# xuhaocuhk/TilinGNN

Measured on AMD Instinct MI355X. Metric: scored tile-nodes/sec (GNN forward), higher is better.
Workload: dtype f32; 1 GPU; TilinGNN.forward on a seeded banded super-graph: 100000 nodes / 1000000 adjacency edges / 1250000 collision edges per GPU, tile_count 2, T=13 edge types, width 32, depth 20, train-mode BatchNorm, graph prep included; n_nodes=100000, n_adj_edges=1000000, n_col_edges=1250000, parallelism=single GPU

## Files before the change

tilingnn_amd/_lib.py:

```python
from __future__ import annotations

import ctypes as C
import os

_HERE = os.path.dirname(os.path.abspath(__file__))
LIB_PATH = os.environ.get("TGNN_LIB_PATH") or os.path.join(_HERE, "libtgnn.so")

ACT_NONE, ACT_LEAKY_RELU, ACT_SIGMOID = 0, 1, 2
BN_MAX_PARTIALS = 512
BN_STAT_ROWS = 4


class TgnnError(RuntimeError):
    code = 0


class ModelDims(C.Structure):
    _fields_ = [("node_features_dim", C.c_int32), ("adj_edge_features_dim", C.c_int32),
                ("network_width", C.c_int32), ("network_depth", C.c_int32), ("output_dim", C.c_int32)]


class Graph(C.Structure):
    _fields_ = [("n_nodes", C.c_int64), ("n_adj_edges", C.c_int64), ("n_col_edges", C.c_int64),
                ("n_types", C.c_int32),
# ... 184 lines not shown
                                           p]),
        "tgnn_nnconv_type_sum": (C.c_int, [p, i64, p, i64, p, p, p, p, i64, i32, i32, p, p]),
        "tgnn_csr_degree": (C.c_int, [p, i64, p, p, p]),
        "tgnn_unsupervised_loss_bwd": (C.c_int, [p, i64, p, i64, i64, p, i64, p, i64, p, i64, f32, f32, f32, p, p, p, i64,
                                                 p, sz, p]),
        "tgnn_f32_to_bf16": (C.c_int, [p, i64, p, p]),
        "tgnn_nnconv64_image_elems": (sz, [i32]),
        "tgnn_nnconv64_bf16_fwd": (C.c_int, [p, i64, p, p, p, p, i32, p, p, i64, i32, p, p, p, pi32, p]),
        "tgnn_nnconv64_bf16_eg_fwd": (C.c_int, [p, i64, p, p, p, i32, p, p, i64, i32, p, p, p, pi32, p]),
        "tgnn_gin64_bf16_fwd": (C.c_int, [p, p, p, p, p, p, p, p, p, p, p, i64, i32, p, p, p, pi32, p]),
        "tgnn_collconv64_bf16_fwd": (C.c_int, [p, p, p, p, p, p, p, p, p, p, p, p, p, p, p, i64, p, p, p, p, p, p]),
        "tgnn_merge_bf16_fwd": (C.c_int, [p, p, p, p, p, i64, i32, p, p]),
        "tgnn_dense_bf16_slots_fwd": (C.c_int, [p, i64, i32, p, p, i64, i32, i32, p, p, p, pi32, p]),
        "tgnn_forward_bf16_workspace_bytes": (sz, [C.POINTER(ModelDims), i64, i32]),
        "tgnn_forward_bf16": (C.c_int, [C.POINTER(ModelDims), C.POINTER(C.c_void_p), p, p, C.POINTER(Graph), i32, p, p, sz, p, p]),
        "tgnn_forward_bf16_begin": (C.c_int, [C.POINTER(ModelDims), C.POINTER(C.c_void_p), p, i64, i32, p, sz, p]),
        "tgnn_rows_gather": (C.c_int, [p, i64, p, i64, i32, p, i64, p]),
        "tgnn_rows_scatter": (C.c_int, [p, p, i64, i32, p, i64, p]),
    }
    for name, (res, args) in sigs.items():
        fn = getattr(lib, name)
        fn.restype, fn.argtypes = res, args
    for name, (res, args) in {"tgnn_debug_spin_fault": (None, [i32]), "tgnn_debug_set_csr_bucket_cap": (i32, [i32]),
                              "tgnn_debug_set_block_caps": (None, [i32, i32])}.items():
        try:
            fn = getattr(lib, name)
        except AttributeError:
            continue
        fn.restype, fn.argtypes = res, args
    return lib


DEBUG_LIB_PATH = os.path.join(_HERE, "libtgnn_debug.so")


def has_debug_hooks() -> bool:
    return hasattr(lib, "tgnn_debug_spin_fault")


lib = _load()
EXPORTED_SYMBOLS = (
    "tgnn_version", "tgnn_last_error", "tgnn_csr_workspace_bytes", "tgnn_csr_build",
    "tgnn_edge_dedup_workspace_bytes", "tgnn_edge_type_dedup", "tgnn_gather_i32", "tgnn_edge_weight_table",
    "tgnn_nnconv_mean_fwd", "tgnn_nnconv_cols_max_columns", "tgnn_nnconv_cols_workspace_bytes",
    "tgnn_nnconv_cols_build", "tgnn_nnconv_cols_max_types", "tgnn_nnconv_weight_image_floats", "tgnn_nnconv_mean_cols_fwd", "tgnn_nnconv_mean_cols_f16_fwd", "tgnn_nnconv_eg_max_groups", "tgnn_nnconv_eg_build", "tgnn_nnconv_mean_eg_fwd",
    "tgnn_ubench_row_gather", "tgnn_mid_entries_words", "tgnn_mid_entries_build", "tgnn_forward_path_counts", "tgnn_set_mid_layout_limit", "tgnn_get_mid_layout_limit", "tgnn_mid_layout_max_nodes",
    "tgnn_spin_error_poll", "tgnn_set_spin_budget_us", "tgnn_persist_fallback", "tgnn_spin_error_peek", "tgnn_gin_fwd", "tgnn_dense_act_fwd", "tgnn_dense_act_slots_fwd", "tgnn_dense_act_slots_f16_fwd", "tgnn_bn_finalize", "tgnn_bn_apply",
# ... 207 lines not shown
```

tilingnn_amd/csrc/graph_prep.hip:

```cpp
#include <atomic>
#include <chrono>
#include <mutex>
#include <vector>

#include "tgnn_common.h"

namespace tgnn {

constexpr int kScanThreads = 256;
constexpr int kScanItems = 8;
constexpr int kScanTile = kScanThreads * kScanItems;

__device__ __forceinline__ int wave_inclusive_scan(int v) {
    const int lane = threadIdx.x & 63;
#pragma unroll
    for (int d = 1; d < 64; d <<= 1) {
        int t = __shfl_up(v, d, 64);
        if (lane >= d) v += t;
    }
    return v;
}

__global__ __launch_bounds__(kScanThreads) void scan_tiles_kernel(const int *in, int *out,
                                                                  int *__restrict__ block_sums, int64_t n) {
// ... 478 lines not shown
    const int n_edge_cols = base[k][n_types];
    for (int c = 0; c < n_edge_cols; ++c) col_slot_src[(c0 + c) * 16 + i] = -1;
    for (int t = i; t < n_types; t += 16) {
        const int m = maxm[k][t];
        for (int r = 0; r < m; ++r)
            col_meta[c0 + base[k][t] + r] = t | (r == 0 ? 1 << 8 : 0) | (r == m - 1 ? 1 << 9 : 0);
    }
    const int deg = e1 - e0;
    col_slot_src[(c0 + n_edge_cols) * 16 + i] = row < n ? __float_as_int((float)(deg > 0 ? deg : 1)) : -1;
    if (i == 0) col_meta[c0 + n_edge_cols] = n_types | (1 << 8) | (1 << 9) | (1 << 10);
    __builtin_amdgcn_fence(__ATOMIC_RELEASE, "wavefront");
    __builtin_amdgcn_wave_barrier();
    for (int t = 0; t < n_types; ++t) cnt[tid][t] = 0;
    for (int e = e0; e < e1; ++e) {
        const int t = col_type[e];
        const int r = cnt[tid][t]++;
        col_slot_src[(c0 + base[k][t] + r) * 16 + i] = col_src[e];
    }
}

constexpr int kEgRoot = 1 << 8;
constexpr int kPrepWordsMagic = 0x600D0001;

template <bool FILL>
__global__ __launch_bounds__(64) void nnconv_eg_kernel(const int *__restrict__ rowptr, const int *__restrict__ col_src,
                                                       const int *__restrict__ col_type, int64_t n, int n_types_host,
                                                       int *__restrict__ tile_grps,
                                                       const int *__restrict__ tile_grp_ptr,
                                                       int2 *__restrict__ grp,
                                                       const int *__restrict__ n_types_dev = nullptr, int max_types = kMaxColTypes,
                                                       int *__restrict__ built_flag = nullptr,
                                                       const int *__restrict__ edge_type = nullptr,
                                                       const int *__restrict__ col_eid = nullptr,
                                                       int *__restrict__ col_type_out = nullptr,
                                                       const int *__restrict__ result_words = nullptr,
                                                       int *__restrict__ host_words = nullptr) {
    if (!FILL && host_words && blockIdx.x == 0 && threadIdx.x < 32) {
        const int v = result_words[threadIdx.x];
        if (threadIdx.x < 31) __hip_atomic_store(host_words + threadIdx.x, v, __ATOMIC_RELAXED, __HIP_MEMORY_SCOPE_SYSTEM);
        __threadfence_system();
        if (threadIdx.x == 31) __hip_atomic_store(host_words + 31, kPrepWordsMagic, __ATOMIC_RELEASE, __HIP_MEMORY_SCOPE_SYSTEM);
    }
    const int n_types = n_types_dev ? *n_types_dev : n_types_host;
    const int64_t n_tiles = (n + kColTileRows - 1) / kColTileRows;
    if (!FILL && col_type_out) {
        const int64_t row0 = (int64_t)blockIdx.x * 64 + threadIdx.x;
        if (row0 < n)
            for (int e = rowptr[row0]; e < rowptr[row0 + 1]; ++e) col_type_out[e] = edge_type[col_eid[e]];
    }
    if (!FILL && blockIdx.x == 0 && threadIdx.x == 0) tile_grps[n_tiles] = 0;
    const int tid = threadIdx.x, k = tid >> 4, i = tid & 15;
    const int64_t row = (int64_t)blockIdx.x * 64 + tid;
    const int64_t tile = (int64_t)blockIdx.x * 4 + k;
    if (n_types > max_types || n_types > kMaxColTypes) {
        if (!FILL && i == 0 && tile < n_tiles) tile_grps[tile] = 0;
        return;
    }
    if (built_flag && blockIdx.x == 0 && threadIdx.x == 0) *built_flag = 1;
    __shared__ unsigned short cnt[64][kMaxColTypes + 1];
    __shared__ unsigned short pre[FILL ? 64 : 1][kMaxColTypes + 1];
    __shared__ int base[4][kMaxColTypes + 1];
    for (int t = 0; t < n_types; ++t) cnt[tid][t] = 0;
    int e0 = 0, e1 = 0;
    if (row < n) { e0 = rowptr[row]; e1 = rowptr[row + 1]; }
    if (!FILL && col_type_out) {
        for (int e = e0; e < e1; ++e) cnt[tid][col_type_out[e]]++;
    } else {
        for (int e = e0; e < e1; ++e) cnt[tid][col_type[e]]++;
    }
    __syncthreads();
    for (int t = i; t < n_types; t += 16) {
        int acc = 0;
        for (int r = 0; r < 16; ++r) {
            if constexpr (FILL) pre[k * 16 + r][t] = (unsigned short)acc;
            acc += cnt[k * 16 + r][t];
        }
        base[k][t] = (acc + 15) >> 4;
    }
    __syncthreads();
    if (i == 0) {
        int acc = 0;
        for (int t = 0; t < n_types; ++t) { const int g = base[k][t]; base[k][t] = acc; acc += g; }
        base[k][n_types] = acc;
        if (!FILL && tile < n_tiles) tile_grps[tile] = acc + 1;
    }
    if (!FILL) return;
    __syncthreads();
    if (tile >= n_tiles) return;
    const int64_t g0 = tile_grp_ptr[tile];
    const int n_edge_grps = base[k][n_types];
    for (int t = 0; t < n_types; ++t)
        for (int g = base[k][t]; g < base[k][t + 1]; ++g) grp[(g0 + g) * 16 + i] = make_int2(-1, t << 16);
    const int deg = e1 - e0;
    grp[(g0 + n_edge_grps) * 16 + i] =
        make_int2(row < n ? __float_as_int((float)(deg > 0 ? deg : 1)) : -1, (n_types | kEgRoot) << 16 | 1 << i);
    __builtin_amdgcn_fence(__ATOMIC_RELEASE, "wavefront");
    __builtin_amdgcn_wave_barrier();
    for (int t = 0; t < n_types; ++t) {
        const int c = cnt[tid][t];
        if (c == 0) continue;
        const int p0 = pre[tid][t], p1 = p0 + c;
        for (int g = p0 >> 4; g <= (p1 - 1) >> 4; ++g) {
            const int lo = max(p0 - 16 * g, 0), hi = min(p1 - 16 * g, 16);
            grp[(g0 + base[k][t] + g) * 16 + i].y = t << 16 | (((1 << hi) - 1) & ~((1 << lo) - 1));
        }
        cnt[tid][t] = 0;
    }
    for (int e = e0; e < e1; ++e) {
        const int t = col_type[e];
        const int p = (unsigned short)(pre[tid][t] + cnt[tid][t]++);
        grp[(g0 + base[k][t] + (p >> 4)) * 16 + (p & 15)].x = col_src[e];
    }
}

constexpr int kSmallPrepThreads = 1024, kSmallPrepMaxNodes = 4096, kSmallPrepMaxBlocks = 16;
constexpr int kSmallPrepLocal = 8192;
constexpr int kSmallPrepGlobal = 8192;
constexpr int kSmallPrepMaxTypes = 1024;

struct SmallPrepArgs {
    const int64_t *adj_ei, *col_ei;
    const float *attr;
    int64_t n, ea, ec;
    int fe, max_col_types;
    int *adj_rowptr, *adj_src, *adj_eid, *adj_type;
    int *edge_type, *type_rep;
    int *col_rowptr, *col_src, *col_eid;
    int *tile_col_ptr, *col_meta, *col_slot_src;
    int *result_host;
    int *tmp;
    int *result;
    unsigned *ctr;
};

__device__ int small_block_scan(int *a, int m, int *wave_tot) {
// ... 421 lines not shown

constexpr int kBkLogMax = 9, kBkRows = 1 << kBkLogMax, kBkMaxBuckets = 4096, kBkThreads = 1024;
constexpr int kBkCap = 15360;
constexpr int kBkCapHalf = 7168;
struct BkSet {
    const int64_t *ei;
    int64_t e;
    int drop_self;
    int *rowptr, *col_src, *col_eid, *err_flag;
    int *rec_eid, *rec_src;
    unsigned short *rec_row;
    int *total_out, *max_deg_out;
};
struct BkArgs {
    BkSet set[2];
    int64_t n, n_src;
    int nb, nblk;
    int lg;
    int cap;
    int cap_lds;
    int *hist;
    const int *tile_off;
    unsigned *scan_ticket;
};
__device__ __forceinline__ int bk_scanned(const BkArgs &A, int64_t i) {
    const int v = A.hist[i];
    return A.tile_off ? v + A.tile_off[i / kScanTile] : v;
}

__global__ __launch_bounds__(kBkThreads) void bk_hist_kernel(BkArgs A) {
    extern __shared__ int bk_h[];
    const BkSet S = A.set[blockIdx.y];
    const int tid = threadIdx.x, blk = blockIdx.x;
    for (int b = tid; b < A.nb; b += kBkThreads) bk_h[b] = 0;
    __syncthreads();
    const int64_t i0 = S.e * blk / A.nblk, i1 = S.e * (blk + 1) / A.nblk;
    for (int64_t i = i0 + tid; i < i1; i += kBkThreads) {
        const int64_t s = S.ei[i], d = S.ei[S.e + i];
        if (s < 0 || s >= A.n_src || d < 0 || d >= A.n) {
            if (S.err_flag) *S.err_flag = 1;
        } else if (!(S.drop_self && s == d)) {
            atomicAdd(&bk_h[d >> A.lg], 1);
        }
    }
    __syncthreads();
    for (int b = tid; b < A.nb; b += kBkThreads) A.hist[((int64_t)blockIdx.y * A.nb + b) * A.nblk + blk] = bk_h[b];
    if (blk == 0 && blockIdx.y == 1 && tid == 0) {
        A.hist[(int64_t)2 * A.nb * A.nblk] = 0;
        if (A.scan_ticket) *A.scan_ticket = 0u;
    }
}

constexpr int kBkChunk = kBkThreads * 8;
__global__ __launch_bounds__(kBkThreads) void bk_scatter_kernel(BkArgs A) {
    extern __shared__ int bk_h[];
    int *cur = bk_h, *lcnt = cur + A.nb, *lstart = lcnt + A.nb, *wtot = lstart + A.nb;
    int *l_eid = wtot + 16, *l_src = l_eid + kBkChunk;
    unsigned short *l_row = reinterpret_cast<unsigned short *>(l_src + kBkChunk), *l_bkt = l_row + kBkChunk;
    const BkSet S = A.set[blockIdx.y];
    const int tid = threadIdx.x, blk = blockIdx.x;
    const int base = bk_scanned(A, (int64_t)blockIdx.y * A.nb * A.nblk);
    for (int b = tid; b < A.nb; b += kBkThreads) cur[b] = bk_scanned(A, ((int64_t)blockIdx.y * A.nb + b) * A.nblk + blk) - base;
    const int64_t i0 = S.e * blk / A.nblk, i1 = S.e * (blk + 1) / A.nblk;
    const int per = (A.nb + kBkThreads - 1) / kBkThreads;
    for (int64_t c0 = i0; c0 < i1; c0 += kBkChunk) {
        for (int b = tid; b < A.nb; b += kBkThreads) lcnt[b] = 0;
        __syncthreads();
        int e_b[8], e_r[8], e_s[8], e_row[8];
#pragma unroll
        for (int u = 0; u < 8; ++u) {
            const int64_t i = c0 + tid + (int64_t)u * kBkThreads;
            e_b[u] = -1;
// ... 208 lines not shown
    hipEvent_t ev = nullptr;
    TGNN_CHECK_HIP(prep_words_event(&ev));
    TGNN_CHECK_HIP(hipEventSynchronize(ev));
    return TGNN_OK;
}

static int bk_blocks(int64_t e_max) {
    int64_t nblk = (e_max + 8191) / 8192;
    return (int)(nblk < 1 ? 1 : (nblk > 256 ? 256 : nblk));
}
static int bk_log_rows(int64_t n, int64_t e_max) {
    return (n <= (int64_t)256 * kBkMaxBuckets && e_max * 256 <= (int64_t)3584 * (n > 0 ? n : 1)) ? 8 : 9;
}
static size_t bk_workspace_bytes(int64_t n, int64_t ea, int64_t ec) {
    const int64_t rows = (int64_t)1 << bk_log_rows(n, ea > ec ? ea : ec);
    const int64_t nb = (n + rows - 1) / rows, nblk = bk_blocks(ea > ec ? ea : ec), cells = 2 * nb * nblk + 1;
    return align_up((size_t)cells * 4, 256) + scan_ws_ints(cells) * 4 + align_up((size_t)(ea > 0 ? ea : 1) * 10, 256) +
           align_up((size_t)(ec > 0 ? ec : 1) * 10, 256) + 2048;
}
static bool bk_fits(int64_t n) { return (n + kBkRows - 1) / kBkRows <= kBkMaxBuckets; }

static int csr_build_pair_bucketed(const int64_t *adj_ei, int64_t ea, const int64_t *col_ei, int64_t ec, int64_t n, int64_t n_src,
                                   int *a_rowptr, int *a_src, int *a_eid, int *a_err, int *c_rowptr, int *c_src, int *c_eid,
                                   int *c_err, int *a_max_deg, int *c_total, void *ws, size_t ws_bytes, hipStream_t s) {
    BkArgs A{};
    A.n = n; A.n_src = n_src;
    A.lg = bk_log_rows(n, ea > ec ? ea : ec);
    A.nb = (int)((n + ((int64_t)1 << A.lg) - 1) >> A.lg);
    A.nblk = bk_blocks(ea > ec ? ea : ec);
    A.cap_lds = A.lg == 8 ? kBkCapHalf : kBkCap;
    A.cap = g_bk_cap.load() < A.cap_lds ? g_bk_cap.load() : A.cap_lds;
    const int64_t cells = (int64_t)2 * A.nb * A.nblk + 1;
    Carver cv(ws, ws_bytes);
    A.hist = cv.take<int>(cells);
    int *scan_ws = cv.take<int>(scan_ws_ints(cells));
    const int64_t es[2] = {ea, ec};
    for (int k = 0; k < 2; ++k) {
        const int64_t e1 = es[k] > 0 ? es[k] : 1;
        unsigned char *rec = cv.take<unsigned char>((size_t)e1 * 10);
        A.set[k].rec_eid = reinterpret_cast<int *>(rec);
        A.set[k].rec_src = reinterpret_cast<int *>(rec + (size_t)e1 * 4);
        A.set[k].rec_row = reinterpret_cast<unsigned short *>(rec + (size_t)e1 * 8);
    }
    A.set[0].ei = adj_ei; A.set[0].e = ea; A.set[0].drop_self = 0;
    A.set[0].rowptr = a_rowptr; A.set[0].col_src = a_src; A.set[0].col_eid = a_eid; A.set[0].err_flag = a_err;
    A.set[1].ei = col_ei; A.set[1].e = ec; A.set[1].drop_self = 1;
    A.set[1].rowptr = c_rowptr; A.set[1].col_src = c_src; A.set[1].col_eid = c_eid; A.set[1].err_flag = c_err;
    A.set[0].max_deg_out = a_max_deg;
// ... 8 lines not shown
    bk_hist_kernel<<<dim3(A.nblk, 2), kBkThreads, lds_h, s>>>(A);
    if (fused_scan)
        scan_tiles_fused_kernel<<<(unsigned)scan_tiles, kScanThreads, 0, s>>>(A.hist, A.hist, scan_ws, const_cast<int *>(A.tile_off), cells,
                                                                             A.scan_ticket);
    else
        exclusive_scan_i32(A.hist, A.hist, cells, scan_ws, s);
    const size_t lds_s = (size_t)(3 * A.nb + 16 + 2 * kBkChunk) * sizeof(int) + (size_t)2 * kBkChunk * sizeof(unsigned short);
    static LdsOptIn site_s;
    TGNN_CHECK_HIP(opt_in_dynamic_lds(bk_scatter_kernel, (int)(160 * 1024 - 256), site_s));
    bk_scatter_kernel<<<dim3(A.nblk, 2), kBkThreads, lds_s, s>>>(A);
    const size_t lds_r = (size_t)(2 * (1 << A.lg) + 1 + 16 + 2 * A.cap_lds) * sizeof(int) + (size_t)A.cap_lds * sizeof(unsigned short);
    static LdsOptIn site;
    TGNN_CHECK_HIP(opt_in_dynamic_lds(bk_rows_kernel, (int)(160 * 1024 - 256), site));
    bk_rows_kernel<<<dim3(A.nb, 2), kBkThreads, lds_r, s>>>(A);
    TGNN_CHECK_LAUNCH();
    return TGNN_OK;
}

}

using namespace tgnn;

#ifdef TGNN_DEBUG
extern "C" int32_t tgnn_debug_set_csr_bucket_cap(int32_t cap) {
    const int prev = g_bk_cap.load();
    if (cap >= 0) g_bk_cap.store(cap > kBkCap ? kBkCap : cap);
    return prev;
}
#endif

extern "C" size_t tgnn_csr_workspace_bytes(int64_t n_nodes, int64_t n_edges) {
    return align_up((size_t)(n_nodes + 1) * 4, 256) + align_up((size_t)(n_edges > 0 ? n_edges : 1) * 4, 256) +
           scan_ws_ints(n_nodes + 1) * 4 + 1024;
}

extern "C" int tgnn_csr_build(const int64_t *edge_index, int64_t n_edges, int64_t n_nodes, int64_t n_src_nodes,
                              int drop_self_loops, int32_t *rowptr, int32_t *col_src, int32_t *col_eid, int32_t *err_flag, void *ws,
                              size_t ws_bytes, tgnn_stream_t stream) {
    DeviceGuard guard__(stream);
    TGNN_CHECK_ARG(n_nodes >= 0 && n_nodes < (1ll << 31) - 1, "n_nodes must fit int32");
    TGNN_CHECK_ARG(n_src_nodes >= n_nodes && n_src_nodes < (1ll << 31) - 1, "n_src_nodes must be >= n_nodes and fit int32");
    TGNN_CHECK_ARG(n_edges >= 0 && n_edges < (1ll << 31) - 1, "n_edges must fit int32");
    TGNN_CHECK_ARG(rowptr && (n_edges == 0 || (edge_index && col_src && col_eid)), "null pointer");
    if (ws_bytes < tgnn_csr_workspace_bytes(n_nodes, n_edges) || !ws) {
        set_error("tgnn_csr_build: workspace too small");
        return TGNN_ERR_WORKSPACE;
// ... 116 lines not shown
    }
    hipStream_t s = static_cast<hipStream_t>(stream);
    const int64_t nt16 = (n_nodes + kColTileRows - 1) / kColTileRows;
    Carver cv(ws, ws_bytes);
    int *tile_cols = cv.take<int>(nt16 + 1);
    int *scan_ws = cv.take<int>(scan_ws_ints(nt16 + 1));
    TGNN_CHECK_HIP(hipMemsetAsync(tile_cols + nt16, 0, 4, s));
    const unsigned blocks = (unsigned)((n_nodes + 63) / 64);
    nnconv_col_kernel<false><<<blocks, 64, 0, s>>>(rowptr, col_src, col_type, n_nodes, n_types, tile_cols, nullptr,
                                                   nullptr, nullptr);
    exclusive_scan_i32(tile_cols, tile_col_ptr, nt16 + 1, scan_ws, s);
    nnconv_col_kernel<true><<<blocks, 64, 0, s>>>(rowptr, col_src, col_type, n_nodes, n_types, nullptr, tile_col_ptr,
                                                  col_meta, col_slot_src);
    TGNN_CHECK_LAUNCH();
    return TGNN_OK;
}

extern "C" int64_t tgnn_nnconv_eg_max_groups(int64_t n_nodes, int64_t n_edges, int32_t n_types) {
    const int64_t ntiles = (n_nodes + kColTileRows - 1) / kColTileRows;
    const int64_t a = n_edges / 16 + ntiles * (int64_t)n_types, b = n_edges;
    return (a < b ? a : b) + ntiles + 32;
}

static void launch_nnconv_eg_build(const int32_t *rowptr, const int32_t *col_src, int32_t *col_type, int64_t n_nodes,
                                   int32_t n_types, const int *n_types_dev, int max_types, int32_t *tile_grps,
                                   int32_t *tile_grp_ptr, int32_t *grp, int *scan_ws, int *built_flag, hipStream_t s,
                                   const int32_t *edge_type = nullptr, const int32_t *col_eid = nullptr,
                                   const int32_t *result_words = nullptr, int32_t *host_words = nullptr) {
    const int64_t nt16 = (n_nodes + kColTileRows - 1) / kColTileRows;
    const unsigned blocks = (unsigned)((n_nodes + 63) / 64);
    nnconv_eg_kernel<false><<<blocks, 64, 0, s>>>(rowptr, col_src, col_type, n_nodes, n_types, tile_grps, nullptr, nullptr,
                                                  n_types_dev, max_types, built_flag, edge_type, col_eid,
                                                  edge_type ? col_type : nullptr, result_words, host_words);
    exclusive_scan_i32(tile_grps, tile_grp_ptr, nt16 + 1, scan_ws, s);
    nnconv_eg_kernel<true><<<blocks, 64, 0, s>>>(rowptr, col_src, col_type, n_nodes, n_types, nullptr, tile_grp_ptr,
                                                 reinterpret_cast<int2 *>(grp), n_types_dev, max_types, nullptr);
}

extern "C" int tgnn_nnconv_eg_build(const int32_t *rowptr, const int32_t *col_src, const int32_t *col_type,
                                    int64_t n_nodes, int32_t n_types, int32_t *tile_grp_ptr, int32_t *grp, void *ws,
                                    size_t ws_bytes, tgnn_stream_t stream) {
    DeviceGuard guard__(stream);
    TGNN_CHECK_ARG(n_nodes >= 1, "n_nodes");
    TGNN_CHECK_ARG(n_types >= 0 && n_types <= kMaxColTypes, "the NNConv edge-group structure supports at most 40 edge types");
    TGNN_CHECK_ARG(rowptr && tile_grp_ptr && grp && ((uintptr_t)grp % 8) == 0, "null / misaligned pointer");
    TGNN_CHECK_ARG(n_types == 0 || (col_src && col_type), "null CSR pointer");
    if (!ws || ws_bytes < tgnn_nnconv_cols_workspace_bytes(n_nodes)) {
        set_error("tgnn_nnconv_eg_build: workspace too small");
        return TGNN_ERR_WORKSPACE;
    }
    hipStream_t s = static_cast<hipStream_t>(stream);
    const int64_t nt16 = (n_nodes + kColTileRows - 1) / kColTileRows;
    Carver cv(ws, ws_bytes);
    int *tile_grps = cv.take<int>(nt16 + 1);
    int *scan_ws = cv.take<int>(scan_ws_ints(nt16 + 1));
    launch_nnconv_eg_build(rowptr, col_src, const_cast<int32_t *>(col_type), n_nodes, n_types, nullptr, kMaxColTypes, tile_grps,
                           tile_grp_ptr, grp, scan_ws, nullptr, s);
    TGNN_CHECK_LAUNCH();
    return TGNN_OK;
// ... 433 lines not shown
    TGNN_CHECK_ARG(!want_eg || (grp && ((uintptr_t)grp % 8) == 0), "edge groups: tile_grp_ptr and an 8-byte aligned grp go together");
    TGNN_CHECK_ARG(want_cols || !(mid_tile_nb && mid_ent), "the mid-size batches are built from the type columns");
    if (!ws || ws_bytes < tgnn_graph_prep_workspace_bytes(n_nodes, n_adj_edges, n_col_edges, fe)) {
        set_error("tgnn_graph_prep: workspace too small");
        return TGNN_ERR_WORKSPACE;
    }
    hipStream_t s = static_cast<hipStream_t>(stream);
    const int64_t emax = n_adj_edges > n_col_edges ? n_adj_edges : n_col_edges;
    Carver cv(ws, ws_bytes);
    const size_t csr_b = tgnn_csr_workspace_bytes(n_nodes, emax), dd_b = tgnn_edge_dedup_workspace_bytes(n_adj_edges, fe),
                 col_b = tgnn_nnconv_cols_workspace_bytes(n_nodes);
    void *ws_csr = cv.take<unsigned char>(csr_b), *ws_dd = cv.take<unsigned char>(dd_b), *ws_col = cv.take<unsigned char>(col_b);
    TGNN_CHECK_HIP(hipMemsetAsync(result, 0, 32 * sizeof(int32_t), s));
    hipStream_t s_side = nullptr;
    hipEvent_t ev_fork = nullptr, ev_join = nullptr;
    if (n_adj_edges > 0 && prep_side_stream(&s_side, &ev_fork, &ev_join) == TGNN_OK) {
        TGNN_CHECK_HIP(hipEventRecord(ev_fork, s));
        TGNN_CHECK_HIP(hipStreamWaitEvent(s_side, ev_fork, 0));
    } else {
        s_side = nullptr;
    }
    int rc;
    bool bucketed = false;
    auto bail = [&](int code) {
        if (s_side && hipEventRecord(ev_join, s_side) == hipSuccess) (void)hipStreamWaitEvent(s, ev_join, 0);
        return code;
    };
    const bool csr_first = n_adj_edges + n_col_edges >= 1000000;
    auto queue_dedup = [&]() -> int {
        if (!s_side) return TGNN_OK;
        rc = edge_type_dedup_listed(adj_edge_attr, n_adj_edges, fe, edge_type, type_rep_edge, result + 0, result + 6, ws_dd, dd_b, s_side);
        if (rc != TGNN_OK) return bail(rc);
        if (hipEventRecord(ev_join, s_side) != hipSuccess) {
            (void)hipStreamSynchronize(s_side);
            set_error("tgnn_graph_prep: hipEventRecord failed");
            return TGNN_ERR_LAUNCH;
        }
        return TGNN_OK;
    };
    if (!csr_first) {
        const int rcd = queue_dedup();
        if (rcd != TGNN_OK) return rcd;
    }
    if (bk_fits(n_nodes) && n_adj_edges < (int64_t(1) << 31) - 1 && n_col_edges < (int64_t(1) << 31) - 1) {
        const size_t bk_b = bk_workspace_bytes(n_nodes, n_adj_edges, n_col_edges);
        void *ws_bk = cv.take<unsigned char>(bk_b);
        rc = csr_build_pair_bucketed(adj_edge_index, n_adj_edges, col_edge_index, n_col_edges, n_nodes, n_src_nodes, adj_rowptr, adj_src,
                                     adj_eid, result + 1, col_rowptr, col_src, col_eid, result + 2, result + 4, result + 3, ws_bk, bk_b, s);
        if (rc != TGNN_OK) return bail(rc);
        bucketed = true;
    } else {
        rc = tgnn_csr_build(adj_edge_index, n_adj_edges, n_nodes, n_src_nodes, 0, adj_rowptr, adj_src, adj_eid, result + 1, ws_csr, csr_b, stream);
        if (rc != TGNN_OK) return bail(rc);
        rc = tgnn_csr_build(col_edge_index, n_col_edges, n_nodes, n_src_nodes, 1, col_rowptr, col_src, col_eid, result + 2, ws_csr, csr_b, stream);
        if (rc != TGNN_OK) return bail(rc);
    }
    if (csr_first) {
        const int rcd = queue_dedup();
        if (rcd != TGNN_OK) return rcd;
    }
    if (s_side) {
        TGNN_CHECK_HIP(hipStreamWaitEvent(s, ev_join, 0));
    } else {
        rc = tgnn_edge_type_dedup(adj_edge_attr, n_adj_edges, fe, edge_type, type_rep_edge, result + 0, ws_dd, dd_b, stream);
        if (rc != TGNN_OK) return rc;
    }
    if (!bucketed) {
        int64_t rb = (n_nodes + 1023) / 1024;
        prep_result_kernel<<<(unsigned)(rb > 256 ? 256 : rb), 256, 0, s>>>(col_rowptr, adj_rowptr, n_nodes, result);
    }
    int32_t *host_words_dev = nullptr;
// ... 2 lines not shown
        void *dptr = nullptr;
        if (hipGetDevice(&dev) == hipSuccess && dev >= 0 && dev < 64 && hipHostGetDevicePointer(&dptr, result_host, 0) == hipSuccess && dptr) {
            if (g_prep_poll[dev]) TGNN_CHECK_HIP(hipDeviceSynchronize());
            host_words_dev = static_cast<int32_t *>(dptr);
            __atomic_store_n(result_host + 31, 0, __ATOMIC_RELEASE);
            g_prep_poll[dev] = result_host;
        } else {
            (void)hipGetLastError();
        }
    }
    if (result_host && !host_words_dev) {
        hipEvent_t ev_words = nullptr;
        TGNN_CHECK_HIP(prep_words_event(&ev_words));
        if (s_side) {
            TGNN_CHECK_HIP(hipEventRecord(ev_fork, s));
            TGNN_CHECK_HIP(hipStreamWaitEvent(s_side, ev_fork, 0));
            TGNN_CHECK_HIP(hipMemcpyAsync(result_host, result, 32 * sizeof(int32_t), hipMemcpyDeviceToHost, s_side));
            TGNN_CHECK_HIP(hipEventRecord(ev_words, s_side));
        } else {
            TGNN_CHECK_HIP(hipMemcpyAsync(result_host, result, 32 * sizeof(int32_t), hipMemcpyDeviceToHost, s));
            TGNN_CHECK_HIP(hipEventRecord(ev_words, s));
        }
    }
    const int64_t nt16 = (n_nodes + kColTileRows - 1) / kColTileRows;
    Carver cc(ws_col, col_b);
    int *tile_cols = cc.take<int>(nt16 + 1);
    int *scan_ws = cc.take<int>(scan_ws_ints(nt16 + 1));
    const unsigned blocks = (unsigned)((n_nodes + 63) / 64);
    const int max_types = tgnn_nnconv_cols_max_types();
    if (want_cols) {
        nnconv_col_kernel<false><<<blocks, 64, 0, s>>>(adj_rowptr, adj_src, adj_type, n_nodes, 0, tile_cols, nullptr, nullptr, nullptr,
                                                       result + 0, max_types, nullptr, n_adj_edges > 0 ? edge_type : nullptr, adj_eid,
                                                       n_adj_edges > 0 ? adj_type : nullptr);
        exclusive_scan_i32(tile_cols, tile_col_ptr, nt16 + 1, scan_ws, s);
        nnconv_col_kernel<true><<<blocks, 64, 0, s>>>(adj_rowptr, adj_src, adj_type, n_nodes, 0, nullptr, tile_col_ptr, col_meta,
                                                      col_slot_src, result + 0, max_types, result + 5);
    }
    if (want_eg) {
        const bool gather_types = !want_cols && n_adj_edges > 0;
        launch_nnconv_eg_build(adj_rowptr, adj_src, adj_type, n_nodes, 0, result + 0, max_types, tile_cols, tile_grp_ptr, grp, scan_ws,
                               result + 10, s, gather_types ? edge_type : nullptr, gather_types ? adj_eid : nullptr,
                               host_words_dev ? result : nullptr, host_words_dev);
    }
    TGNN_CHECK_LAUNCH();
    if (mid_tile_nb && mid_ent) {
        rc = tgnn_mid_entries_build(tile_col_ptr, col_meta, col_slot_src, n_nodes, result + 5, mid_tile_nb, mid_ent, result + 8, stream);
        if (rc != TGNN_OK) return rc;
    }
    return TGNN_OK;
}
```

Before: 54.39 million nodes/s.

## Restructure edge-group graph prep into wave-per-tile count and fill kernels with fused scan

Replaces the per-row edge-group count/fill kernels with a wave-per-tile design. The count kernel tallies types with LDS atomics over coalesced edge passes, and its last block (chosen by an atomic ticket) performs the tile-offset exclusive scan, removing a separate scan launch. The fill kernel ranks edges with ballot/popcount, assembles each tile's groups in LDS, and writes them out coalesced, replacing scattered per-row global writes. Tiles with too many edges or groups fall back to a row-wise path. The cost is higher code complexity and a ticket word that the bucketed CSR build must reset.

```diff
diff --git a/tilingnn_amd/_lib.py b/tilingnn_amd/_lib.py
--- a/tilingnn_amd/_lib.py
+++ b/tilingnn_amd/_lib.py
@@ -230,7 +230,7 @@
         fn = getattr(lib, name)
         fn.restype, fn.argtypes = res, args
     for name, (res, args) in {"tgnn_debug_spin_fault": (None, [i32]), "tgnn_debug_set_csr_bucket_cap": (i32, [i32]),
-                              "tgnn_debug_set_block_caps": (None, [i32, i32])}.items():
+                              "tgnn_debug_set_block_caps": (None, [i32, i32]), "tgnn_debug_set_eg_fast_edges": (i32, [i32])}.items():
         try:
             fn = getattr(lib, name)
         except AttributeError:
diff --git a/tilingnn_amd/csrc/graph_prep.hip b/tilingnn_amd/csrc/graph_prep.hip
--- a/tilingnn_amd/csrc/graph_prep.hip
+++ b/tilingnn_amd/csrc/graph_prep.hip
@@ -524,95 +524,310 @@
 constexpr int kEgRoot = 1 << 8;
 constexpr int kPrepWordsMagic = 0x600D0001;
 
+constexpr int kEgCountThreads = 1024, kEgCountWaves = kEgCountThreads / 64;
+constexpr int kEgThreads = 256, kEgWaves = kEgThreads / 64;
+constexpr int kEgPass = 256;
+constexpr int kEgStageGrps = 40;
+constexpr int kEgFastEdges = 2048;
+constexpr int kEgTypeSlots = 48;
+constexpr int kEgRowwiseBytes = 2 * 16 * (kMaxColTypes + 1) * 2 + (kMaxColTypes + 1) * 4;
+constexpr int kEgRowwiseInt2 = (kEgRowwiseBytes + 7) / 8;
+static_assert(kEgRowwiseInt2 <= kEgStageGrps * 16 && kEgTypeSlots > kMaxColTypes && (16 * (kMaxColTypes + 1) * 2) % 4 == 0, "staging");
+constexpr int kEgScanPer = 16, kEgScanMax = kEgCountThreads * kEgScanPer;
+static std::atomic<int> g_eg_fast_edges{kEgFastEdges};
+
+__device__ __forceinline__ void wave_lds_sync() {
+    __builtin_amdgcn_fence(__ATOMIC_ACQ_REL, "wavefront");
+    __builtin_amdgcn_wave_barrier();
+}
+
 template <bool FILL>
-__global__ __launch_bounds__(64) void nnconv_eg_kernel(const int *__restrict__ rowptr, const int *__restrict__ col_src,
-                                                       const int *__restrict__ col_type, int64_t n, int n_types_host,
-                                                       int *__restrict__ tile_grps,
-                                                       const int *__restrict__ tile_grp_ptr,
-                                                       int2 *__restrict__ grp,
-                                                       const int *__restrict__ n_types_dev = nullptr, int max_types = kMaxColTypes,
-                                                       int *__restrict__ built_flag = nullptr,
-                                                       const int *__restrict__ edge_type = nullptr,
-                                                       const int *__restrict__ col_eid = nullptr,
-                                                       int *__restrict__ col_type_out = nullptr,
-                                                       const int *__restrict__ result_words = nullptr,
-                                                       int *__restrict__ host_words = nullptr) {
-    if (!FILL && host_words && blockIdx.x == 0 && threadIdx.x < 32) {
-        const int v = result_words[threadIdx.x];
-        if (threadIdx.x < 31) __hip_atomic_store(host_words + threadIdx.x, v, __ATOMIC_RELAXED, __HIP_MEMORY_SCOPE_SYSTEM);
-        __threadfence_system();
-        if (threadIdx.x == 31) __hip_atomic_store(host_words + 31, kPrepWordsMagic, __ATOMIC_RELEASE, __HIP_MEMORY_SCOPE_SYSTEM);
-    }
+__device__ __forceinline__ int eg_tile_rowwise(int2 *stage, const int lane, const int64_t tile, const int *__restrict__ rowptr,
+                                               const int *__restrict__ col_src, const int *col_type,
+                                               const int *__restrict__ edge_type, const int *__restrict__ col_eid, const int64_t n,
+                                               const int n_types, const int64_t g0, int2 *__restrict__ grp) {
+    typedef unsigned short Row16[kMaxColTypes + 1];
+    Row16 *cnt = reinterpret_cast<Row16 *>(stage);
+    Row16 *pre = cnt + 16;
+    int *base = reinterpret_cast<int *>(pre + 16);
+    const int i = lane;
+    const bool on = lane < 16;
+    const int64_t row = tile * kColTileRows + i;
+    int e0 = 0, e1 = 0;
+    if (on) {
+        for (int t = 0; t < n_types; ++t) cnt[i][t] = 0;
+        if (row < n) { e0 = rowptr[row]; e1 = rowptr[row + 1]; }
+        for (int e = e0; e < e1; ++e) {
+            const int t = edge_type ? edge_type[col_eid[e]] : col_type[e];
+            if ((unsigned)t < (unsigned)n_types) cnt[i][t]++;
+        }
+    }
+    wave_lds_sync();
+    if (on)
+        for (int t = i; t < n_types; t += 16) {
+            int acc = 0;
+            for (int r = 0; r < 16; ++r) {
+                pre[r][t] = (unsigned short)acc;
+                acc += cnt[r][t];
+            }
+            base[t] = (acc + 15) >> 4;
+        }
+    wave_lds_sync();
+    if (lane == 0) {
+        int acc = 0;
+        for (int t = 0; t < n_types; ++t) { const int g = base[t]; base[t] = acc; acc += g; }
+        base[n_types] = acc;
+    }
+    wave_lds_sync();
+    const int n_edge_grps = base[n_types];
+    if constexpr (FILL) {
+        if (on) {
+            for (int t = 0; t < n_types; ++t)
+                for (int g = base[t]; g < base[t + 1]; ++g) grp[(g0 + g) * 16 + i] = make_int2(-1, t << 16);
+            const int deg = e1 - e0;
+            grp[(g0 + n_edge_grps) * 16 + i] =
+                make_int2(row < n ? __float_as_int((float)(deg > 0 ? deg : 1)) : -1, (n_types | kEgRoot) << 16 | 1 << i);
+            __builtin_amdgcn_fence(__ATOMIC_RELEASE, "wavefront");
+            __builtin_amdgcn_wave_barrier();
+            for (int t = 0; t < n_types; ++t) {
+                const int c = cnt[i][t];
+                if (c == 0) continue;
+                const int p0 = pre[i][t], p1 = p0 + c;
+                for (int g = p0 >> 4; g <= (p1 - 1) >> 4; ++g) {
+                    const int lo = max(p0 - 16 * g, 0), hi = min(p1 - 16 * g, 16);
+                    grp[(g0 + base[t] + g) * 16 + i].y = t << 16 | (((1 << hi) - 1) & ~((1 << lo) - 1));
+                }
+                cnt[i][t] = 0;
+            }
+            for (int e = e0; e < e1; ++e) {
+                const int t = col_type[e];
+                if ((unsigned)t >= (unsigned)n_types) continue;
+                const int p = (unsigned short)(pre[i][t] + cnt[i][t]++);
+                grp[(g0 + base[t] + (p >> 4)) * 16 + (p & 15)].x = col_src[e];
+            }
+        }
+    }
+    return n_edge_grps + 1;
+}
+
+__global__ __launch_bounds__(kEgCountThreads) void nnconv_eg_count_kernel(const int *__restrict__ rowptr, const int *col_type, int64_t n,
+                                                                     int n_types_host, int *__restrict__ tile_grps,
+                                                                     int *__restrict__ tile_grp_ptr, unsigned *__restrict__ ticket,
+                                                                     const int *__restrict__ n_types_dev, int max_types,
+                                                                     int *__restrict__ built_flag, const int *__restrict__ edge_type,
+                                                                     const int *__restrict__ col_eid, int *col_type_out,
+                                                                     const int *__restrict__ result_words, int *__restrict__ host_words,
+                                                                     int fast_edges) {
+    __shared__ int s_cnt[kEgCountWaves][kEgTypeSlots];
+    __shared__ int2 s_stage[kEgCountWaves][kEgRowwiseInt2];
+    __shared__ int s_wave_tot[kEgCountWaves];
+    __shared__ unsigned s_ticket;
+    const int tid = threadIdx.x, lane = tid & 63, wave = tid >> 6;
     const int n_types = n_types_dev ? *n_types_dev : n_types_host;
     const int64_t n_tiles = (n + kColTileRows - 1) / kColTileRows;
-    if (!FILL && col_type_out) {
-        const int64_t row0 = (int64_t)blockIdx.x * 64 + threadIdx.x;
-        if (row0 < n)
-            for (int e = rowptr[row0]; e < rowptr[row0 + 1]; ++e) col_type_out[e] = edge_type[col_eid[e]];
-    }
-    if (!FILL && blockIdx.x == 0 && threadIdx.x == 0) tile_grps[n_tiles] = 0;
-    const int tid = threadIdx.x, k = tid >> 4, i = tid & 15;
-    const int64_t row = (int64_t)blockIdx.x * 64 + tid;
-    const int64_t tile = (int64_t)blockIdx.x * 4 + k;
-    if (n_types > max_types || n_types > kMaxColTypes) {
-        if (!FILL && i == 0 && tile < n_tiles) tile_grps[tile] = 0;
+    const bool built = !(n_types > max_types || n_types > kMaxColTypes);
+    int words = 0;
+    if (host_words && blockIdx.x == 0 && wave == 0) words = result_words[lane & 31];
+    if (blockIdx.x == 0 && tid == 0) {
+        if (host_words) {
+#pragma unroll
+            for (int k = 0; k < 31; ++k)
+                __hip_atomic_store(host_words + k, (built && result_words + k == built_flag) ? 1 : __builtin_amdgcn_readlane(words, k),
+                                   __ATOMIC_RELAXED, __HIP_MEMORY_SCOPE_SYSTEM);
+            __threadfence_system();
+            __hip_atomic_store(host_words + 31, kPrepWordsMagic, __ATOMIC_RELEASE, __HIP_MEMORY_SCOPE_SYSTEM);
+        }
+        if (built && built_flag) *built_flag = 1;
+        __hip_atomic_store(tile_grps + n_tiles, 0, __ATOMIC_RELAXED, __HIP_MEMORY_SCOPE_AGENT);
+    }
+    const int64_t tile = (int64_t)blockIdx.x * kEgCountWaves + wave;
+    if (tile < n_tiles) {
+        const int64_t r = tile * kColTileRows + lane;
+        const int rpv = lane <= kColTileRows ? rowptr[r < n ? r : n] : 0;
+        const int t0 = __builtin_amdgcn_readlane(rpv, 0), t1 = __builtin_amdgcn_readlane(rpv, kColTileRows);
+        const bool fast = built && t1 - t0 <= fast_edges;
+        int *cnt = s_cnt[wave];
+        if (lane < kEgTypeSlots) cnt[lane] = 0;
+        wave_lds_sync();
+        if (col_type_out || fast) {
+            for (int b = t0; b < t1; b += kEgPass) {
+                int ty[kEgPass / 64];
+                if (col_type_out) {
+                    int eid[kEgPass / 64];
+#pragma unroll
+                    for (int k = 0; k < kEgPass / 64; ++k) {
+                        const int e = b + k * 64 + lane;
+                        eid[k] = e < t1 ? col_eid[e] : -1;
+                    }
+#pragma unroll
+                    for (int k = 0; k < kEgPass / 64; ++k) ty[k] = eid[k] >= 0 ? edge_type[eid[k]] : -1;
+#pragma unroll
+                    for (int k = 0; k < kEgPass / 64; ++k) {
+                        const int e = b + k * 64 + lane;
+                        if (e < t1) col_type_out[e] = ty[k];
+                    }
+                } else {
+#pragma unroll
+                    for (int k = 0; k < kEgPass / 64; ++k) {
+                        const int e = b + k * 64 + lane;
+                        ty[k] = e < t1 ? col_type[e] : -1;
+                    }
+                }
+                if (fast) {
+#pragma unroll
+                    for (int k = 0; k < kEgPass / 64; ++k)
+                        if ((unsigned)ty[k] < (unsigned)n_types) atomicAdd(&cnt[ty[k]], 1);
+                }
+            }
+        }
+        int ngrp = 0;
+        if (fast) {
+            wave_lds_sync();
+            int g = lane < n_types ? (cnt[lane] + 15) >> 4 : 0;
+#pragma unroll
+            for (int d = 32; d >= 1; d >>= 1) g += __shfl_xor(g, d, 64);
+            ngrp = g + 1;
+        } else if (built) {
+            ngrp = eg_tile_rowwise<false>(s_stage[wave], lane, tile, rowptr, nullptr, col_type, col_type_out ? edge_type : nullptr, col_eid, n,
+                                          n_types, 0, nullptr);
+        }
+        if (lane == 0) __hip_atomic_store(tile_grps + tile, ngrp, __ATOMIC_RELAXED, __HIP_MEMORY_SCOPE_AGENT);
+    }
+    if (!ticket) return;
+    asm volatile("s_waitcnt vmcnt(0)" ::: "memory");
+    __syncthreads();
+    if (tid == 0) s_ticket = __hip_atomic_fetch_add(ticket, 1u, __ATOMIC_RELAXED, __HIP_MEMORY_SCOPE_AGENT);
+    __syncthreads();
+    if (s_ticket != gridDim.x - 1) return;
+    const int m = (int)n_tiles + 1, per = (m + kEgCountThreads - 1) / kEgCountThreads;
+    const int b = tid * per, e = min(b + per, m);
+    int v[kEgScanPer];
+    int sum = 0;
+#pragma unroll
+    for (int k = 0; k < kEgScanPer; ++k) {
+        v[k] = (k < per && b + k < e) ? __hip_atomic_load(tile_grps + b + k, __ATOMIC_RELAXED, __HIP_MEMORY_SCOPE_AGENT) : 0;
+        sum += v[k];
+    }
+    const int incl = wave_inclusive_scan(sum);
+    if (lane == 63) s_wave_tot[wave] = incl;
+    __syncthreads();
+    int run = incl - sum;
+    for (int w = 0; w < wave; ++w) run += s_wave_tot[w];
+#pragma unroll
+    for (int k = 0; k < kEgScanPer; ++k) {
+        if (k < per && b + k < e) tile_grp_ptr[b + k] = run;
+        run += v[k];
+    }
+    if (tid == 0) __hip_atomic_store(ticket, 0u, __ATOMIC_RELAXED, __HIP_MEMORY_SCOPE_AGENT);
+}
+
+__global__ __launch_bounds__(kEgThreads) void nnconv_eg_fill_kernel(const int *__restrict__ rowptr, const int *__restrict__ col_src,
+                                                                    const int *__restrict__ col_type, int64_t n, int n_types_host,
+                                                                    const int *__restrict__ tile_grp_ptr, int2 *__restrict__ grp,
+                                                                    const int *__restrict__ n_types_dev, int max_types, int fast_edges) {
+    __shared__ int2 s_rec[kEgWaves][kEgStageGrps * 16];
+    __shared__ int s_cnt[kEgWaves][kEgTypeSlots];
+    const int tid = threadIdx.x, lane = tid & 63, wave = tid >> 6;
+    const int n_types = n_types_dev ? *n_types_dev : n_types_host;
+    const int64_t n_tiles = (n + kColTileRows - 1) / kColTileRows;
+    if (n_types > max_types || n_types > kMaxColTypes) return;
+    const int64_t tile = (int64_t)blockIdx.x * kEgWaves + wave;
+    if (tile >= n_tiles) return;
+    const int64_t r = tile * kColTileRows + lane;
+    const int rpv = lane <= kColTileRows ? rowptr[r < n ? r : n] : 0;
+    const int gv = lane < 2 ? tile_grp_ptr[tile + lane] : 0;
+    const int t0 = __builtin_amdgcn_readlane(rpv, 0), t1 = __builtin_amdgcn_readlane(rpv, kColTileRows);
+    const int64_t g0 = __builtin_amdgcn_readlane(gv, 0);
+    const int ng = __builtin_amdgcn_readlane(gv, 1) - (int)g0;
+    int2 *rec = s_rec[wave];
+    if (t1 - t0 > fast_edges || ng > kEgStageGrps || ng < 1) {
+        eg_tile_rowwise<true>(rec, lane, tile, rowptr, col_src, col_type, nullptr, nullptr, n, n_types, g0, grp);
         return;
     }
-    if (built_flag && blockIdx.x == 0 && threadIdx.x == 0) *built_flag = 1;
-    __shared__ unsigned short cnt[64][kMaxColTypes + 1];
-    __shared__ unsigned short pre[FILL ? 64 : 1][kMaxColTypes + 1];
-    __shared__ int base[4][kMaxColTypes + 1];
-    for (int t = 0; t < n_types; ++t) cnt[tid][t] = 0;
-    int e0 = 0, e1 = 0;
-    if (row < n) { e0 = rowptr[row]; e1 = rowptr[row + 1]; }
-    if (!FILL && col_type_out) {
-        for (int e = e0; e < e1; ++e) cnt[tid][col_type_out[e]]++;
-    } else {
-        for (int e = e0; e < e1; ++e) cnt[tid][col_type[e]]++;
-    }
-    __syncthreads();
-    for (int t = i; t < n_types; t += 16) {
-        int acc = 0;
-        for (int r = 0; r < 16; ++r) {
-            if constexpr (FILL) pre[k * 16 + r][t] = (unsigned short)acc;
-            acc += cnt[k * 16 + r][t];
-        }
-        base[k][t] = (acc + 15) >> 4;
-    }
-    __syncthreads();
-    if (i == 0) {
-        int acc = 0;
-        for (int t = 0; t < n_types; ++t) { const int g = base[k][t]; base[k][t] = acc; acc += g; }
-        base[k][n_types] = acc;
-        if (!FILL && tile < n_tiles) tile_grps[tile] = acc + 1;
-    }
-    if (!FILL) return;
-    __syncthreads();
-    if (tile >= n_tiles) return;
-    const int64_t g0 = tile_grp_ptr[tile];
-    const int n_edge_grps = base[k][n_types];
-    for (int t = 0; t < n_types; ++t)
-        for (int g = base[k][t]; g < base[k][t + 1]; ++g) grp[(g0 + g) * 16 + i] = make_int2(-1, t << 16);
-    const int deg = e1 - e0;
-    grp[(g0 + n_edge_grps) * 16 + i] =
-        make_int2(row < n ? __float_as_int((float)(deg > 0 ? deg : 1)) : -1, (n_types | kEgRoot) << 16 | 1 << i);
-    __builtin_amdgcn_fence(__ATOMIC_RELEASE, "wavefront");
-    __builtin_amdgcn_wave_barrier();
-    for (int t = 0; t < n_types; ++t) {
-        const int c = cnt[tid][t];
-        if (c == 0) continue;
-        const int p0 = pre[tid][t], p1 = p0 + c;
-        for (int g = p0 >> 4; g <= (p1 - 1) >> 4; ++g) {
-            const int lo = max(p0 - 16 * g, 0), hi = min(p1 - 16 * g, 16);
-            grp[(g0 + base[k][t] + g) * 16 + i].y = t << 16 | (((1 << hi) - 1) & ~((1 << lo) - 1));
-        }
-        cnt[tid][t] = 0;
-    }
-    for (int e = e0; e < e1; ++e) {
-        const int t = col_type[e];
-        const int p = (unsigned short)(pre[tid][t] + cnt[tid][t]++);
-        grp[(g0 + base[k][t] + (p >> 4)) * 16 + (p & 15)].x = col_src[e];
-    }
+    int rp[kColTileRows];
+#pragma unroll
+    for (int j = 1; j < kColTileRows; ++j) rp[j] = __builtin_amdgcn_readlane(rpv, j);
+    int *cnt = s_cnt[wave];
+    if (lane < kEgTypeSlots) cnt[lane] = 0;
+    wave_lds_sync();
+    int ty[kEgPass / 64], sr[kEgPass / 64];
+    auto load_pass = [&](const int b) {
+#pragma unroll
+        for (int k = 0; k < kEgPass / 64; ++k) {
+            const int e = b + k * 64 + lane;
+            const int t = e < t1 ? col_type[e] : -1;
+            ty[k] = (unsigned)t < (unsigned)n_types ? t : -1;
+            sr[k] = e < t1 ? col_src[e] : -1;
+        }
+    };
+    load_pass(t0);
+#pragma unroll
+    for (int k = 0; k < kEgPass / 64; ++k)
+        if (ty[k] >= 0) atomicAdd(&cnt[ty[k]], 1);
+    for (int b = t0 + kEgPass; b < t1; b += kEgPass) {
+#pragma unroll
+        for (int k = 0; k < kEgPass / 64; ++k) {
+            const int e = b + k * 64 + lane;
+            const int t = e < t1 ? col_type[e] : -1;
+            if ((unsigned)t < (unsigned)n_types) atomicAdd(&cnt[t], 1);
+        }
+    }
+    wave_lds_sync();
+    const int gt = lane < n_types ? (cnt[lane] + 15) >> 4 : 0;
+    const int first = wave_inclusive_scan(gt) - gt;
+    wave_lds_sync();
+    if (lane <= n_types) cnt[lane] = first;
+    wave_lds_sync();
+    const int n_edge_grps = min(cnt[n_types], ng - 1);
+    for (int tb = 0; tb < n_types; tb += 4) {
+        const int t = tb + (lane >> 4), j = lane & 15;
+        if (t < n_types) {
+            const int ga = cnt[t], gb = min(cnt[t + 1], n_edge_grps);
+            for (int g = ga; g < gb; ++g) rec[g * 16 + j] = make_int2(-1, t << 16);
+        }
+    }
+    {
+        const int deg = __shfl_down(rpv, 1, 64) - rpv;
+        if (lane < kColTileRows)
+            rec[(ng - 1) * 16 + lane] =
+                make_int2(r < n ? __float_as_int((float)(deg > 0 ? deg : 1)) : -1, (n_types | kEgRoot) << 16 | 1 << lane);
+    }
+    wave_lds_sync();
+    int seen = 0;
+    const unsigned long long below = (1ull << lane) - 1ull;
+    for (int b = t0; b < t1; b += kEgPass) {
+        if (b != t0) load_pass(b);
+        int p[kEgPass / 64] = {};
+        for (int t = 0; t < n_types; ++t) {
+            int before = __builtin_amdgcn_readlane(seen, t);
+#pragma unroll
+            for (int k = 0; k < kEgPass / 64; ++k) {
+                const bool mine = ty[k] == t;
+                const unsigned long long same = __ballot(mine);
+                if (mine) p[k] = before + __popcll(same & below);
+                before += __popcll(same);
+            }
+            if (lane == t) seen = before;
+        }
+#pragma unroll
+        for (int k = 0; k < kEgPass / 64; ++k) {
+            if (b + k * 64 >= t1) break;
+            const int e = b + k * 64 + lane;
+            int row = 0;
+#pragma unroll
+            for (int j = 1; j < kColTileRows; ++j) row += e >= rp[j] ? 1 : 0;
+            if (ty[k] >= 0) {
+                const int g = cnt[ty[k]] + (p[k] >> 4), sl = p[k] & 15;
+                if (g < n_edge_grps) {
+                    rec[g * 16 + sl].x = sr[k];
+                    atomicOr(&rec[g * 16 + row].y, 1 << sl);
+                }
+            }
+        }
+    }
+    wave_lds_sync();
+    int2 *out = grp + g0 * 16;
+    for (int i = lane; i < ng * 16; i += 64) out[i] = rec[i];
 }
 
 constexpr int kSmallPrepThreads = 1024, kSmallPrepMaxNodes = 4096, kSmallPrepMaxBlocks = 16;
@@ -1080,6 +1295,7 @@
     int *hist;
     const int *tile_off;
     unsigned *scan_ticket;
+    unsigned *eg_ticket;
 };
 __device__ __forceinline__ int bk_scanned(const BkArgs &A, int64_t i) {
     const int v = A.hist[i];
@@ -1106,6 +1322,7 @@
     if (blk == 0 && blockIdx.y == 1 && tid == 0) {
         A.hist[(int64_t)2 * A.nb * A.nblk] = 0;
         if (A.scan_ticket) *A.scan_ticket = 0u;
+        if (A.eg_ticket) *A.eg_ticket = 0u;
     }
 }
 
@@ -1360,8 +1577,10 @@
 
 static int csr_build_pair_bucketed(const int64_t *adj_ei, int64_t ea, const int64_t *col_ei, int64_t ec, int64_t n, int64_t n_src,
                                    int *a_rowptr, int *a_src, int *a_eid, int *a_err, int *c_rowptr, int *c_src, int *c_eid,
-                                   int *c_err, int *a_max_deg, int *c_total, void *ws, size_t ws_bytes, hipStream_t s) {
+                                   int *c_err, int *a_max_deg, int *c_total, void *ws, size_t ws_bytes, hipStream_t s,
+                                   unsigned *eg_ticket = nullptr) {
     BkArgs A{};
+    A.eg_ticket = eg_ticket;
     A.n = n; A.n_src = n_src;
     A.lg = bk_log_rows(n, ea > ec ? ea : ec);
     A.nb = (int)((n + ((int64_t)1 << A.lg) - 1) >> A.lg);
@@ -1416,6 +1635,11 @@
 using namespace tgnn;
 
 #ifdef TGNN_DEBUG
+extern "C" int32_t tgnn_debug_set_eg_fast_edges(int32_t cap) {
+    const int prev = g_eg_fast_edges.load();
+    if (cap >= 0) g_eg_fast_edges.store(cap > kEgFastEdges ? kEgFastEdges : cap);
+    return prev;
+}
 extern "C" int32_t tgnn_debug_set_csr_bucket_cap(int32_t cap) {
     const int prev = g_bk_cap.load();
     if (cap >= 0) g_bk_cap.store(cap > kBkCap ? kBkCap : cap);
@@ -1578,19 +1802,26 @@
     return (a < b ? a : b) + ntiles + 32;
 }
 
+static unsigned *eg_ticket_word(void *ws_col, int64_t nt16) {
+    char *scan_ws = static_cast<char *>(ws_col) + align_up((size_t)(nt16 + 1) * 4, 256);
+    return reinterpret_cast<unsigned *>(scan_ws) + scan_ws_ints(nt16 + 1) - 32;
+}
+
 static void launch_nnconv_eg_build(const int32_t *rowptr, const int32_t *col_src, int32_t *col_type, int64_t n_nodes,
                                    int32_t n_types, const int *n_types_dev, int max_types, int32_t *tile_grps,
                                    int32_t *tile_grp_ptr, int32_t *grp, int *scan_ws, int *built_flag, hipStream_t s,
                                    const int32_t *edge_type = nullptr, const int32_t *col_eid = nullptr,
-                                   const int32_t *result_words = nullptr, int32_t *host_words = nullptr) {
+                                   const int32_t *result_words = nullptr, int32_t *host_words = nullptr, unsigned *ticket = nullptr) {
     const int64_t nt16 = (n_nodes + kColTileRows - 1) / kColTileRows;
-    const unsigned blocks = (unsigned)((n_nodes + 63) / 64);
-    nnconv_eg_kernel<false><<<blocks, 64, 0, s>>>(rowptr, col_src, col_type, n_nodes, n_types, tile_grps, nullptr, nullptr,
-                                                  n_types_dev, max_types, built_flag, edge_type, col_eid,
-                                                  edge_type ? col_type : nullptr, result_words, host_words);
-    exclusive_scan_i32(tile_grps, tile_grp_ptr, nt16 + 1, scan_ws, s);
-    nnconv_eg_kernel<true><<<blocks, 64, 0, s>>>(rowptr, col_src, col_type, n_nodes, n_types, nullptr, tile_grp_ptr,
-                                                 reinterpret_cast<int2 *>(grp), n_types_dev, max_types, nullptr);
+    const unsigned blocks = (unsigned)((nt16 + kEgWaves - 1) / kEgWaves), cblocks = (unsigned)((nt16 + kEgCountWaves - 1) / kEgCountWaves);
+    const int fast_edges = g_eg_fast_edges.load(std::memory_order_relaxed);
+    const bool fused_scan = ticket && nt16 + 1 <= kEgScanMax;
+    nnconv_eg_count_kernel<<<cblocks, kEgCountThreads, 0, s>>>(rowptr, col_type, n_nodes, n_types, tile_grps, tile_grp_ptr,
+                                                        fused_scan ? ticket : nullptr, n_types_dev, max_types, built_flag, edge_type, col_eid,
+                                                        edge_type ? col_type : nullptr, result_words, host_words, fast_edges);
+    if (!fused_scan) exclusive_scan_i32(tile_grps, tile_grp_ptr, nt16 + 1, scan_ws, s);
+    nnconv_eg_fill_kernel<<<blocks, kEgThreads, 0, s>>>(rowptr, col_src, col_type, n_nodes, n_types, tile_grp_ptr,
+                                                       reinterpret_cast<int2 *>(grp), n_types_dev, max_types, fast_edges);
 }
 
 extern "C" int tgnn_nnconv_eg_build(const int32_t *rowptr, const int32_t *col_src, const int32_t *col_type,
@@ -2070,6 +2301,8 @@
     }
     int rc;
     bool bucketed = false;
+    const int64_t nt16 = (n_nodes + kColTileRows - 1) / kColTileRows;
+    unsigned *eg_ticket = nullptr;
     auto bail = [&](int code) {
         if (s_side && hipEventRecord(ev_join, s_side) == hipSuccess) (void)hipStreamWaitEvent(s, ev_join, 0);
         return code;
@@ -2094,7 +2327,8 @@
         const size_t bk_b = bk_workspace_bytes(n_nodes, n_adj_edges, n_col_edges);
         void *ws_bk = cv.take<unsigned char>(bk_b);
         rc = csr_build_pair_bucketed(adj_edge_index, n_adj_edges, col_edge_index, n_col_edges, n_nodes, n_src_nodes, adj_rowptr, adj_src,
-                                     adj_eid, result + 1, col_rowptr, col_src, col_eid, result + 2, result + 4, result + 3, ws_bk, bk_b, s);
+                                     adj_eid, result + 1, col_rowptr, col_src, col_eid, result + 2, result + 4, result + 3, ws_bk, bk_b, s,
+                                     want_eg ? (eg_ticket = eg_ticket_word(ws_col, nt16)) : nullptr);
         if (rc != TGNN_OK) return bail(rc);
         bucketed = true;
     } else {
@@ -2143,7 +2377,6 @@
             TGNN_CHECK_HIP(hipEventRecord(ev_words, s));
         }
     }
-    const int64_t nt16 = (n_nodes + kColTileRows - 1) / kColTileRows;
     Carver cc(ws_col, col_b);
     int *tile_cols = cc.take<int>(nt16 + 1);
     int *scan_ws = cc.take<int>(scan_ws_ints(nt16 + 1));
@@ -2161,7 +2394,7 @@
         const bool gather_types = !want_cols && n_adj_edges > 0;
         launch_nnconv_eg_build(adj_rowptr, adj_src, adj_type, n_nodes, 0, result + 0, max_types, tile_cols, tile_grp_ptr, grp, scan_ws,
                                result + 10, s, gather_types ? edge_type : nullptr, gather_types ? adj_eid : nullptr,
-                               host_words_dev ? result : nullptr, host_words_dev);
+                               host_words_dev ? result : nullptr, host_words_dev, eg_ticket);
     }
     TGNN_CHECK_LAUNCH();
     if (mid_tile_nb && mid_ent) {
```

Result: no change. 54.59 million nodes/s, median of 6 (+0.4%).
